# williamyang98/DAB-Radio

Hardware: AMD Instinct MI355X
Metric: dab_mode1_frames_per_sec (higher is better)
Workload: dtype f32

## Files before the change

### dab-radio_amd/csrc/viterbi_lanes.hip

```cpp
#include <hip/hip_runtime.h>
#include <stdint.h>

#include "dabgpu_internal.h"
#include "viterbi_pk16.h"

namespace dabgpu {

__host__ __device__ constexpr int vl_rotl6(int v, int s) { return ((v << s) | (v >> (6 - s))) & 63; }
__host__ __device__ constexpr int vl_idx(int n, int q) { return ((n >> (q + 1)) << q) | (n & ((1 << q) - 1)); }

template <int QN>
__device__ __forceinline__ void vl_gather(const s2 (&D)[32], uint32_t& w0, uint32_t& w1) {
    constexpr int S = (QN + 3) % 6;
    uint32_t G[16];
#pragma unroll
    for (int g = 0; g < 16; g++) {
        const int base = ((g >> 3) << 5) | (g & 7);
        const int r_lo = vl_idx(vl_rotl6(base, S), QN), r_hi = vl_idx(vl_rotl6(base | 16, S), QN);
        G[g] = __builtin_amdgcn_perm(as_u32(D[r_hi]), as_u32(D[r_lo]), 0x0B0A0908u);
    }
    uint32_t a0 = G[0], a1 = G[8];
#pragma unroll
    for (int k = 1; k < 8; k++) {
        a0 = vl_bfi(0x01010101u << k, G[k], a0);
        a1 = vl_bfi(0x01010101u << k, G[8 + k], a1);
    }
    w0 = a0; w1 = a1;
}

template <int Q, int TIE>
__device__ __forceinline__ void vl_step(const s2 (&M)[32], s2 (&N)[32], uint32_t ysym, int k508, uint32_t& w0, uint32_t& w1) {
    s2 C[8], D[32];
    {
        using map = vl_costmap<vl_flip(Q)>;
        constexpr int WF[4] = {map::wF(0, 1, 1, 1), map::wF(1, 1, 1, 1), map::wF(2, 1, 1, 1), map::wF(3, 1, 1, 1)};
        constexpr int WX[4] = {map::wX(0, 1, 1, 1), map::wX(1, 1, 1, 1), map::wX(2, 1, 1, 1), map::wX(3, 1, 1, 1)};
        vl_cost_table<vl_flip(Q), true>(ysym, WF, WX, k508, C);
    }
    if constexpr (Q < 5) {
#pragma unroll
        for (int i = 0; i < 16; i++) {
            const int s = vl_sigma(vl_ins_zero(i, Q));
            const s2 c1 = C[s], c2 = C[7 - s];
            const s2 t1 = addm<TIE>(M[i], c1), t2 = addm<TIE>(M[i + 16], c2);
            const s2 t3 = addm<TIE>(M[i], c2), t4 = addm<TIE>(M[i + 16], c1);
            N[2 * i] = min16(t1, t2);
            N[2 * i + 1] = min16(t3, t4);
            D[2 * i] = TIE ? satsub16(t1, t2) : satsub16(t2, t1);
            D[2 * i + 1] = TIE ? satsub16(t3, t4) : satsub16(t4, t3);
        }
    } else {
#pragma unroll
        for (int b = 0; b < 32; b++) {
            const int s = vl_sigma(b);
            const s2 lower = addm<TIE>(__builtin_shufflevector(M[b], M[b], 0, 0), C[s]);
            const s2 upper = addm<TIE>(__builtin_shufflevector(M[b], M[b], 1, 1), C[7 - s]);
            N[b] = min16(lower, upper);
            D[b] = TIE ? satsub16(lower, upper) : satsub16(upper, lower);
        }
    }
    vl_gather<(Q + 1) % 6>(D, w0, w1);
    if constexpr (TIE != 0) { w0 = ~w0; w1 = ~w1; }
}

__device__ __forceinline__ void vl_renorm(s2 (&N)[32], uint32_t& total) {
    if ((int)N[0].x >= (int)(60455 - 32768)) {
        s2 red[16];
#pragma unroll
        for (int r = 0; r < 16; r++) red[r] = min16(N[r], N[r + 16]);
#pragma unroll
        for (int w = 8; w >= 1; w >>= 1) {
#pragma unroll
            for (int r = 0; r < w; r++) red[r] = min16(red[r], red[r + w]);
        }
        s2 mn = red[0];
        mn = min16(mn, swap16(mn));
        const uint32_t mu = ((uint32_t)(uint16_t)mn.x) ^ 0x8000u;
        const s2 sub = as_s2(mu | (mu << 16));
#pragma unroll
        for (int r = 0; r < 32; r++) N[r] = sub16(N[r], sub);
        total += mu;
    }
}

__device__ __forceinline__ uint2 vl_sched_entry(int t, const uint32_t* seg_pi, const uint32_t* seg_steps, uint32_t in_rows,
                                                const dabgpu_vit_tables* __restrict__ tables) {
    int sstart = 0, in0 = 0, pi = 8, k = 0;
    for (; k < 4; k++) {
        const int len = (int)seg_steps[k];
        if (t < sstart + len) { pi = (int)seg_pi[k]; break; }
        in0 += (len >> 3) * (8 + (int)seg_pi[k]);
        sstart += len;
    }
    const int sis = t - sstart;
    const uint16_t e = tables->pi_tab[pi * 8 + (sis & 7)];
    const uint32_t cnt = e & 0xFFu, kk = (uint32_t)(in0 + (sis >> 3) * (8 + pi)) + (uint32_t)(e >> 8);
    const uint32_t keep = cnt >= 4u ? 0xFFFFFFFFu : ((1u << (8u * cnt)) - 1u);
    uint2 r;
    r.x = min(kk >> 2, in_rows - 2u);
    r.y = ((0x03020100u + (kk & 3u) * 0x01010101u) & keep) | (0x0C0C0C0Cu & ~keep);
    return r;
}

constexpr int VL_OBYTES = 100;

template <int TIE, int VL_WAVES, int OCC = 4>
__global__ __launch_bounds__(64 * VL_WAVES) __attribute__((amdgpu_waves_per_eu(OCC, OCC)))
void vit_lanes_kernel(const dabgpu_vit_group* __restrict__ groups, int n_groups, const dabgpu_cw_desc* __restrict__ descs,
                      const uint32_t* __restrict__ sym, uint32_t* __restrict__ dec, dabgpu_cw_result* __restrict__ results,
                      const dabgpu_vit_tables* __restrict__ tables, const uint2* __restrict__ sched)
{
    __shared__ unsigned char prbs[512];
    __shared__ unsigned short crc_tab[256];
    __shared__ unsigned char obuf[VL_WAVES][64][VL_OBYTES];
    const int lane = threadIdx.x & 63;
    for (int e = threadIdx.x; e < 512; e += 64 * VL_WAVES) prbs[e] = tables->prbs[e];
    for (int e = threadIdx.x; e < 256; e += 64 * VL_WAVES) {
        unsigned v = (unsigned)e << 8;
        for (int qq = 0; qq < 8; qq++) v = (v & 0x8000u) ? (((v << 1) ^ 0x1021u) & 0xFFFFu) : ((v << 1) & 0xFFFFu);
        crc_tab[e] = (unsigned short)v;
    }
    __syncthreads();
    const int wvi = __builtin_amdgcn_readfirstlane((int)(threadIdx.x >> 6));
    const int group = (int)blockIdx.x * VL_WAVES + wvi;
    if (group >= n_groups) return;

    const dabgpu_vit_group Gd = groups[group];
    const int T = (int)Gd.n_steps;
    const bool valid = lane < (int)Gd.count;
    const size_t cw = (size_t)Gd.first + (size_t)Gd.stride * (size_t)(valid ? lane : 0);
    const dabgpu_cw_desc Dd = descs[cw];
    const bool live = valid && Dd.n_steps != 0;

    const uint32_t* grp_sym = sym + Gd.sym_off;
    uint32_t* grp_dec = dec + Gd.dec_off;

    const int q0 = (6 - T % 6) % 6;
    s2 M[32], N[32];
    {
        const uint32_t ss = Dd.start_state & 63u;
        const uint32_t r0 = ((ss >> (q0 + 1)) << q0) | (ss & ((1u << q0) - 1u)), h0 = (ss >> q0) & 1u;
        const uint32_t non = (5080u ^ 0x8000u), st = 0x8000u;
#pragma unroll
        for (int r = 0; r < 32; r++) {
            const uint32_t lo = ((uint32_t)r == r0 && h0 == 0) ? st : non, hi = ((uint32_t)r == r0 && h0 == 1) ? st : non;
            M[r] = as_s2(lo | (hi << 16));
        }
    }
    uint32_t total = 0;
    int k508 = 508;
    asm volatile("" : "+v"(k508));
    const uint2* sch = sched + Gd.sched_off;
    const uint32_t lane4 = 4u * (uint32_t)lane, lane16 = 16u * (uint32_t)lane;
#define VL_PAIR(Q, TT, YA, YB)                                                                        \
    {                                                                                                 \
        uint4 wv;                                                                                     \
        vl_step<Q, TIE>(M, N, YA, k508, wv.x, wv.y);                                                        \
        vl_renorm(N, total);                                                                          \
        vl_step<(Q) + 1, TIE>(N, M, YB, k508, wv.z, wv.w);                                                  \
        vl_renorm(M, total);                                                                          \
        __builtin_nontemporal_store(u4v{wv.x, wv.y, wv.z, wv.w},                                      \
                                    reinterpret_cast<u4v*>(reinterpret_cast<char*>(grp_dec + (size_t)((TT) >> 1) * 256) + lane16)); \
    }
#define VL_ROWS(LO, HI, SEL, TT)                                                                      \
    {                                                                                                 \
        const uint2 e_ = sch[TT];                                                                     \
        const char* rp_ = reinterpret_cast<const char*>(grp_sym + (size_t)e_.x * 64);                 \
        LO = *reinterpret_cast<const uint32_t*>(rp_ + lane4);                                         \
        HI = *reinterpret_cast<const uint32_t*>(rp_ + 256 + lane4);                                   \
        SEL = e_.y;                                                                                   \
    }
    int t = 0;
    if (q0 == 2) {
        uint32_t a0, a1, b0, b1, sa, sb;
        VL_ROWS(a0, a1, sa, t) VL_ROWS(b0, b1, sb, t + 1)
        VL_PAIR(2, t, __builtin_amdgcn_perm(a1, a0, sa), __builtin_amdgcn_perm(b1, b0, sb))
        t += 2;
    }
    if (q0 != 0) {
        uint32_t a0, a1, b0, b1, sa, sb;
        VL_ROWS(a0, a1, sa, t) VL_ROWS(b0, b1, sb, t + 1)
        VL_PAIR(4, t, __builtin_amdgcn_perm(a1, a0, sa), __builtin_amdgcn_perm(b1, b0, sb))
        t += 2;
    }
    uint32_t nlo[6], nhi[6], nsel[6];
#pragma unroll
    for (int q = 0; q < 6; q++) VL_ROWS(nlo[q], nhi[q], nsel[q], t + q)
    for (; t < T; t += 6) {
        uint32_t y[6];
#pragma unroll
        for (int q = 0; q < 6; q++) y[q] = __builtin_amdgcn_perm(nhi[q], nlo[q], nsel[q]);
#pragma unroll
        for (int q = 0; q < 6; q++) VL_ROWS(nlo[q], nhi[q], nsel[q], t + 6 + q)
        VL_PAIR(0, t, y[0], y[1])
        VL_PAIR(2, t + 2, y[2], y[3])
        VL_PAIR(4, t + 4, y[4], y[5])
    }
#undef VL_ROWS
#undef VL_PAIR

    const uint32_t es = Dd.end_state & 63u;
    uint32_t endm = 0;
#pragma unroll
    for (int r = 0; r < 32; r++) endm = ((es >> 1) == (uint32_t)r) ? as_u32(M[r]) : endm;
    endm = (((es & 1u) ? (endm >> 16) : endm) & 0xFFFFu) ^ 0x8000u;

    __builtin_amdgcn_fence(__ATOMIC_RELEASE, "workgroup");
    __builtin_amdgcn_s_waitcnt(0);

    const bool raw = (Dd.flags & DABGPU_CW_RAW) != 0;
    unsigned char* out = reinterpret_cast<unsigned char*>(Dd.d_out);
    const int n_out = (T - 6) >> 3;
    const bool crc_lds = Dd.n_crc_blocks != 0 && n_out <= VL_OBYTES;
    unsigned char* const ob = &obuf[wvi][lane][0];
    uint32_t pos = ((es >> 3) | (es << 3)) & 63u;
    constexpr int CB = 24;
    uint32_t cx[CB], cy[CB];
    for (int th = T - 1; th >= 6; th -= CB) {
#pragma unroll
        for (int v = 0; v < CB / 2; v++) {
            const int pr = (th >> 1) - v;
            const u4v q4 = __builtin_nontemporal_load(reinterpret_cast<const u4v*>(reinterpret_cast<const char*>(grp_dec + (size_t)(pr < 0 ? 0 : pr) * 256) + lane16));
            cx[2 * v] = q4.z; cy[2 * v] = q4.w; cx[2 * v + 1] = q4.x; cy[2 * v + 1] = q4.y;
        }
#pragma unroll
        for (int ub = 0; ub < CB; ub += 8) {
            if (th - ub >= 6) {
                uint32_t acc = 0;
#pragma unroll
                for (int u = ub; u < ub + 8; u++) {
                    const uint32_t word = (pos & 32u) ? cy[u] : cx[u];
                    const uint32_t d = (word >> (pos & 31u)) & 1u;
                    const int b = (3 + u) % 6;
                    pos = (pos & ~(1u << b)) | (d << b);
                    acc |= d << (u - ub);
                }
                const int k = (th - ub - 7 - 6) >> 3;
                const unsigned char pb = raw ? (unsigned char)0 : prbs[k % VL_PRBS];
                if (live) out[k] = (unsigned char)(acc ^ pb);
                if (crc_lds) ob[k] = (unsigned char)(acc ^ pb);
            }
        }
    }

    uint32_t crc_mask = 0;
    if (live && Dd.n_crc_blocks) {
        if (!crc_lds) {
            __builtin_amdgcn_fence(__ATOMIC_RELEASE, "workgroup");
            __builtin_amdgcn_s_waitcnt(0);
        }
        const int blk_bytes = n_out / (int)Dd.n_crc_blocks;
        for (int b = 0; b < (int)Dd.n_crc_blocks && b < 32; b++) {
            unsigned crc = 0xFFFFu, rx;
            if (crc_lds) {
                const unsigned char* fib = ob + b * blk_bytes;
                for (int i = 0; i < blk_bytes - 2; i++) crc = ((crc << 8) ^ crc_tab[((crc >> 8) ^ fib[i]) & 0xFFu]) & 0xFFFFu;
                rx = ((unsigned)fib[blk_bytes - 2] << 8) | fib[blk_bytes - 1];
            } else {
                const unsigned char* fib = out + b * blk_bytes;
                for (int i = 0; i < blk_bytes - 2; i++)
                    crc = ((crc << 8) ^ crc_tab[((crc >> 8) ^ __builtin_nontemporal_load(&fib[i])) & 0xFFu]) & 0xFFFFu;
                rx = ((unsigned)__builtin_nontemporal_load(&fib[blk_bytes - 2]) << 8) | __builtin_nontemporal_load(&fib[blk_bytes - 1]);
            }
            crc ^= 0xFFFFu;
            if (rx == crc) crc_mask |= 1u << b;
        }
    }
    if (valid) {
        dabgpu_cw_result R;
        R.path_error = live ? (uint64_t)total + endm : 0;
        R.crc_ok_mask = crc_mask;
        R.n_out_bytes = live ? (uint32_t)n_out : 0u;
        *reinterpret_cast<dabgpu_cw_result*>(reinterpret_cast<char*>(results + cw) + Gd.res_delta) = R;
    }
}


__device__ __forceinline__ uint32_t vl_clamp4(uint32_t w) {
    const uint32_t t = w ^ 0x80808080u;
    const uint32_t nz = ((t & 0x7F7F7F7Fu) + 0x7F7F7F7Fu) | t;
    return w + ((~nz & 0x80808080u) >> 7);
}

__global__ __launch_bounds__(256)
void vit_prep_kernel(const dabgpu_vit_group* __restrict__ groups, const dabgpu_cw_desc* __restrict__ descs, uint32_t* __restrict__ sym)
{
    __shared__ uint32_t tile[VL_TILE][65];
    const int tid = threadIdx.x, lane = tid & 63, wv = tid >> 6;
    const dabgpu_vit_group Gd = groups[blockIdx.x];
    const int j0 = blockIdx.y * VL_TILE;
    if (j0 >= (int)Gd.in_rows) return;
    const unsigned n_in = dabgpu_vit_in_bytes(Gd.seg_pi, Gd.seg_steps);
    const unsigned i0 = 4u * (unsigned)(j0 + lane);
    for (int c = wv; c < 64; c += 4) {
        uint32_t packed = 0;
        const bool have = c < (int)Gd.count;
        const dabgpu_cw_desc Dd = descs[(size_t)Gd.first + (size_t)Gd.stride * (size_t)(have ? c : 0)];
        uint32_t aoff = 0;
        unsigned ish = 0;
        if (Dd.n_slots != 0) {
            const int age = 15 - (int)(__brev((unsigned)lane & 15u) >> 28);
            int slot = (int)Dd.newest_slot - age;
            if (slot < 0) slot += (int)Dd.n_slots;
            const int fr = slot / (int)Dd.cifs_per_frame, ci = slot - fr * (int)Dd.cifs_per_frame;
            aoff = (uint32_t)fr * Dd.frame_stride + (uint32_t)ci * Dd.cif_stride;
            if (Dd.flags & DABGPU_CW_CLASSED) { aoff += ((unsigned)lane & 15u) * (Dd.cif_stride >> 4); ish = 4; }
        }
        const int8_t* src = reinterpret_cast<const int8_t*>(Dd.d_src);
#pragma unroll
        for (int r = 0; r < 4; r++) {
            const unsigned i = i0 + (unsigned)r;
            const uint32_t off = (uint32_t)__shfl((int)aoff, (int)(i & 15u));
            if (have && Dd.n_steps != 0 && i < n_in) {
                int yv = src[(size_t)off + (i >> ish)];
                yv = max(yv, -127);
                packed |= ((uint32_t)yv & 0xFFu) << (8 * r);
            }
        }
        tile[lane][c] = packed;
    }
    __syncthreads();
    uint32_t* dst = sym + Gd.sym_off;
    for (int s = wv; s < VL_TILE; s += 4) {
        if (j0 + s < (int)Gd.in_rows) dst[(size_t)(j0 + s) * 64 + lane] = tile[s][lane];
    }
}

__global__ __launch_bounds__(256)
void vit_prep_direct_kernel(const dabgpu_vit_group* __restrict__ groups, const dabgpu_cw_desc* __restrict__ descs, uint32_t* __restrict__ sym)
{
    __shared__ uint32_t rows[64][65];
    const int tid = threadIdx.x, lane = tid & 63, wv = tid >> 6;
    const dabgpu_vit_group Gd = groups[blockIdx.x];
    const int j0 = blockIdx.y * VL_TILE;
    if (j0 >= (int)Gd.in_rows) return;
    const int n_in = (int)dabgpu_vit_in_bytes(Gd.seg_pi, Gd.seg_steps);
    typedef const __attribute__((address_space(1))) unsigned char* gptr;
    u4v v[4];
#pragma unroll
    for (int h = 0; h < 4; h++) {
        const int q = tid + 256 * h, c = q >> 4, ch = q & 15;
        v[h] = u4v{0u, 0u, 0u, 0u};
        if (c < (int)Gd.count) {
            const dabgpu_cw_desc* Dd = descs + ((size_t)Gd.first + (size_t)Gd.stride * (size_t)c);
            const int o = 4 * j0 + 16 * ch;
            if (Dd->n_steps != 0 && o < n_in) {
                const gptr p = (gptr)(uintptr_t)Dd->d_src + o;
                if (o + 16 <= n_in) v[h] = *(const __attribute__((address_space(1))) u4v*)p;
                else {
                    const __attribute__((address_space(1))) uint32_t* pw = (const __attribute__((address_space(1))) uint32_t*)p;
                    v[h].x = pw[0];
                    if (o + 8 <= n_in) v[h].y = pw[1];
                    if (o + 12 <= n_in) v[h].z = pw[2];
                }
            }
        }
    }
#pragma unroll
    for (int h = 0; h < 4; h++) {
        const int q = tid + 256 * h, c = q >> 4, ch = q & 15;
        rows[c][4 * ch] = v[h].x; rows[c][4 * ch + 1] = v[h].y; rows[c][4 * ch + 2] = v[h].z; rows[c][4 * ch + 3] = v[h].w;
    }
    __syncthreads();
    uint32_t* dst = sym + Gd.sym_off;
    for (int s = wv; s < VL_TILE; s += 4) {
        if (j0 + s < (int)Gd.in_rows) dst[(size_t)(j0 + s) * 64 + lane] = vl_clamp4(rows[lane][s]);
    }
}

constexpr int VR_ROWS = 19, VR_CHUNKS = 16, VR_PITCH = VR_CHUNKS * 16 + 16;
__global__ __launch_bounds__(256)
void vit_prep_ring4_kernel(const dabgpu_vit_group* __restrict__ groups, const dabgpu_cw_desc* __restrict__ descs, uint32_t* __restrict__ sym)
{
    __shared__ uint32_t tile[VL_TILE][65];
    __shared__ __attribute__((aligned(16))) unsigned char rows[2][VR_ROWS][VR_PITCH];
    const int tid = threadIdx.x, rowi = tid & 63, c = tid >> 6;
    const dabgpu_vit_group Gd = groups[blockIdx.x];
    const int j0 = blockIdx.y * VL_TILE;
    if (j0 >= (int)Gd.in_rows) return;
    const int n_in = (int)dabgpu_vit_in_bytes(Gd.seg_pi, Gd.seg_steps);
    const int i_lo = 4 * j0, i_hi = min(i_lo + 4 * VL_TILE, n_in);
    int lds_off[4];
    bool in[4];
#pragma unroll
    for (int r = 0; r < 4; r++) {
        const unsigned i = (unsigned)(i_lo + 4 * rowi + r);
        const int age = 15 - (int)(__brev(i & 15u) >> 28);
        lds_off[r] = (c - age + 15) * VR_PITCH + (4 * rowi + r);
        in[r] = (int)i < i_hi;
    }
    auto fetch = [&](int k, uint4 (&v)[2]) {
        const bool have = 4 * k < (int)Gd.count;
        const dabgpu_cw_desc Dd = descs[(size_t)Gd.first + (size_t)Gd.stride * (size_t)(have ? 4 * k : 0)];
        const bool on = have && Dd.n_steps != 0;
        const unsigned char* src = reinterpret_cast<const unsigned char*>(Dd.d_src);
#pragma unroll
        for (int h = 0; h < 2; h++) {
            const int q = tid + 256 * h, row = q >> 4, ch = q & 15;
            v[h] = make_uint4(0, 0, 0, 0);
            if (on && row < VR_ROWS && i_lo + 16 * ch < i_hi) {
                int slot = (int)Dd.newest_slot - 15 + row;
                if (slot < 0) slot += (int)Dd.n_slots;
                if (slot >= (int)Dd.n_slots) slot -= (int)Dd.n_slots;
                const size_t off = (size_t)(slot >> 2) * Dd.frame_stride + (size_t)(slot & 3) * Dd.cif_stride + (size_t)(i_lo + 16 * ch);
                v[h] = *reinterpret_cast<const uint4*>(src + off);
            }
        }
    };
    auto stash = [&](int buf, const uint4 (&v)[2]) {
#pragma unroll
        for (int h = 0; h < 2; h++) {
            const int q = tid + 256 * h, row = q >> 4, ch = q & 15;
            if (row < VR_ROWS) *reinterpret_cast<uint4*>(&rows[buf][row][16 * ch]) = v[h];
        }
    };
    uint4 v[4][2];
    fetch(0, v[0]); fetch(1, v[1]); fetch(2, v[2]); fetch(3, v[3]);
    stash(0, v[0]);
    __syncthreads();
#pragma unroll
    for (int k = 0; k < 16; k++) {
        if (k + 4 < 16) fetch(k + 4, v[k & 3]);
        const unsigned char* rb = &rows[k & 1][0][0];
        uint32_t packed = 0;
#pragma unroll
        for (int r = 0; r < 4; r++) {
            if (in[r]) {
                int yv = (int)(signed char)rb[lds_off[r]];
                yv = max(yv, -127);
                packed |= ((uint32_t)yv & 0xFFu) << (8 * r);
            }
        }
        tile[rowi][4 * k + c] = packed;
        if (k + 1 < 16) stash((k + 1) & 1, v[(k + 1) & 3]);
        __syncthreads();
    }
    uint32_t* dst = sym + Gd.sym_off;
    const int lane = tid & 63, wv = tid >> 6;
    for (int s = wv; s < VL_TILE; s += 4) {
        if (j0 + s < (int)Gd.in_rows) dst[(size_t)(j0 + s) * 64 + lane] = tile[s][lane];
    }
}

constexpr int VC_ROWS = 256, VC_ENS = 4;
constexpr int VC_PITCH = 2 * 64 + 16;
constexpr int VC_CIF_PITCH = 16 * VC_PITCH + 16;
constexpr int VC_ENS_PITCH = 4 * VC_CIF_PITCH;
__global__ __launch_bounds__(256)
void vit_prep_ring4c_kernel(const dabgpu_vit_group* __restrict__ groups, const dabgpu_cw_desc* __restrict__ descs, uint32_t* __restrict__ sym,
                            uint32_t groups_per_sub, uint32_t n_lane_sub)
{
    __shared__ __attribute__((aligned(16))) unsigned char ring[VC_ENS * VC_ENS_PITCH];
    const int tid = threadIdx.x;
    unsigned g_idx = blockIdx.x >> 2;
    int qg = (int)(blockIdx.x & 3);
    if (groups_per_sub != 0) {
        const unsigned x = blockIdx.x & 7, j = blockIdx.x >> 3;
        const unsigned li = j % n_lane_sub, u = (j / n_lane_sub) * 8 + x;
        if (u >= 4 * groups_per_sub) return;
        g_idx = li * groups_per_sub + (u >> 2);
        qg = (int)(u & 3);
    }
    const dabgpu_vit_group Gd = groups[g_idx];
    const int n_in = (int)dabgpu_vit_in_bytes(Gd.seg_pi, Gd.seg_steps);
    typedef const __attribute__((address_space(1))) unsigned char* gptr;
    gptr src[VC_ENS];
    unsigned newest[VC_ENS], n_slots = 16, frame_stride = 0, cif_stride = 0;
    bool on[VC_ENS], any = false;
    int phi = 0;
#pragma unroll
    for (int e = 0; e < VC_ENS; e++) {
        const int ens = VC_ENS * qg + e;
        const bool have = 4 * ens < (int)Gd.count;
        const dabgpu_cw_desc Dd = descs[(size_t)Gd.first + (size_t)Gd.stride * (size_t)(have ? 4 * ens : 0)];
        on[e] = have && Dd.n_steps != 0;
        src[e] = (gptr)(uintptr_t)Dd.d_src;
        newest[e] = Dd.newest_slot;
        if (on[e] && !any) {
            any = true; n_slots = Dd.n_slots; frame_stride = Dd.frame_stride; cif_stride = Dd.cif_stride;
            phi = (int)((uintptr_t)Dd.d_src & 63);
        }
    }
    if (!any) return;
    const int piece = tid >> 2, chunk = tid & 3, l_c16 = piece & 15;
    const int l_rel = (piece >> 4) - (15 - (int)(__brev((unsigned)l_c16) >> 28));
    size_t l_off[VC_ENS];
#pragma unroll
    for (int e = 0; e < VC_ENS; e++) {
        int slot = (int)newest[e] + l_rel;
        if (slot < 0) slot += (int)n_slots;
        if (slot >= (int)n_slots) slot -= (int)n_slots;
        l_off[e] = (size_t)(slot >> 2) * frame_stride + (size_t)(slot & 3) * cif_stride + (size_t)l_c16 * (cif_stride >> 4) + (size_t)(16 * chunk) - (size_t)phi;
    }
    unsigned char* const l_lds = ring + (piece >> 4) * VC_CIF_PITCH + l_c16 * VC_PITCH + 16 * chunk;

    const int real_rows = (n_in + 3) >> 2;
    const int n_tiles = (real_rows + VC_ROWS - 1) / VC_ROWS;
    const int last = (((n_in - 1) >> 4) + phi) >> 6;
    auto tile_hi = [&](int st) { return min(st + (phi ? 1 : 0), last); };
    u4v v[VC_ENS];
    auto fetch = [&](int line) {
#pragma unroll
        for (int e = 0; e < VC_ENS; e++) {
            v[e] = u4v{0u, 0u, 0u, 0u};
            if (on[e]) v[e] = *(const __attribute__((address_space(1))) u4v*)(src[e] + (l_off[e] + (size_t)(64 * line)));
        }
    };
    auto stash = [&](int line) {
#pragma unroll
        for (int e = 0; e < VC_ENS; e++) *reinterpret_cast<u4v*>(l_lds + e * VC_ENS_PITCH + (line & 1) * 64) = v[e];
    };
    int loaded = -1;
    bool pend = false;
    const int e = (tid >> 2) & 3, co = tid & 3;
    const uint32_t* const wb = reinterpret_cast<const uint32_t*>(ring) + e * (VC_ENS_PITCH / 4) + co * (VC_CIF_PITCH / 4);
    uint32_t* const obase = sym + Gd.sym_off + 16 * qg + 4 * e + co;
    for (int st = 0; st < n_tiles; st++) {
        if (pend) { stash(loaded); pend = false; }
        while (loaded < tile_hi(st)) { loaded++; fetch(loaded); stash(loaded); }
        __syncthreads();
        if (st + 1 < n_tiles && loaded < tile_hi(st + 1)) { loaded++; fetch(loaded); pend = true; }
#pragma unroll
        for (int it = 0; it < 4; it++) {
            const int m = (tid >> 4) + 16 * it, q = m & 3, cb = m >> 2;
            const int col = (64 * st + 4 * cb + phi) & 127;
            const uint32_t* wp = wb + (4 * q) * (VC_PITCH / 4) + (col >> 2);
            const uint32_t A = wp[0], B = wp[VC_PITCH / 4], C = wp[2 * (VC_PITCH / 4)], D = wp[3 * (VC_PITCH / 4)];
            const uint32_t T0 = __builtin_amdgcn_perm(B, A, 0x05010400u), T1 = __builtin_amdgcn_perm(B, A, 0x07030602u);
            const uint32_t U0 = __builtin_amdgcn_perm(D, C, 0x05010400u), U1 = __builtin_amdgcn_perm(D, C, 0x07030602u);
            const uint32_t O[4] = {__builtin_amdgcn_perm(U0, T0, 0x05040100u), __builtin_amdgcn_perm(U0, T0, 0x07060302u),
                                   __builtin_amdgcn_perm(U1, T1, 0x05040100u), __builtin_amdgcn_perm(U1, T1, 0x07060302u)};
            const int jb = VC_ROWS * st + 16 * cb + q;
#pragma unroll
            for (int mm = 0; mm < 4; mm++) {
                const int j = jb + 4 * mm;
                if (j < real_rows) obase[(size_t)j * 64] = vl_clamp4(O[mm]);
            }
        }
        __syncthreads();
    }
}

__global__ void vit_groups_uniform_kernel(dabgpu_vit_group* groups, size_t n_cw, uint32_t n_steps, uint32_t alloc_steps, uint32_t in_rows,
                                          uint32_t pi0, uint32_t st0, uint32_t pi1, uint32_t st1, uint32_t pi2, uint32_t st2,
                                          uint32_t pi3, uint32_t st3, dabgpu_vit_group_base base)
{
    const size_t g = (size_t)blockIdx.x * blockDim.x + threadIdx.x;
    if (g * 64 >= n_cw) return;
    dabgpu_vit_group G = {};
    G.first = base.first + (uint32_t)(g * 64); G.stride = 1;
    G.count = (uint32_t)((n_cw - g * 64 < 64) ? (n_cw - g * 64) : 64);
    G.n_steps = n_steps; G.alloc_steps = alloc_steps;
    G.seg_pi[0] = pi0; G.seg_steps[0] = st0; G.seg_pi[1] = pi1; G.seg_steps[1] = st1;
    G.seg_pi[2] = pi2; G.seg_steps[2] = st2; G.seg_pi[3] = pi3; G.seg_steps[3] = st3;
    G.in_rows = in_rows;
    G.sched_off = base.sched_off;
    G.sym_off = base.sym_off + g * (size_t)in_rows * 64;
    G.dec_off = base.dec_off + g * (size_t)alloc_steps * 128;
    G.res_delta = base.res_delta;
    groups[g] = G;
}

__global__ void vit_groups_msc_kernel(dabgpu_vit_group* groups, const dabgpu_msc_plan* plans, const uint64_t* lane_subs,
                                      int n_lane_sub, int n_sub, size_t n_ens, uint32_t groups_per_sub, uint32_t sched_stride)
{
    const size_t g = (size_t)blockIdx.x * blockDim.x + threadIdx.x;
    if (g >= (size_t)n_lane_sub * groups_per_sub) return;
    const int li = (int)(g / groups_per_sub);
    const uint32_t gq = (uint32_t)(g - (size_t)li * groups_per_sub);
    const int s = (int)lane_subs[3 * li];
    const dabgpu_msc_plan P = plans[s];
    const size_t n_j = n_ens * 4;
    dabgpu_vit_group G = {};
    G.first = (uint32_t)((size_t)s + (size_t)n_sub * 64 * gq); G.stride = (uint32_t)n_sub;
    G.count = (uint32_t)((n_j - (size_t)gq * 64 < 64) ? (n_j - (size_t)gq * 64) : 64);
    G.n_steps = P.n_steps;
    G.alloc_steps = dabgpu_vit_alloc_steps(P.n_steps);
    for (int k = 0; k < 4; k++) { G.seg_pi[k] = P.seg_pi[k]; G.seg_steps[k] = P.seg_steps[k]; }
    G.in_rows = dabgpu_vit_in_rows(dabgpu_vit_in_bytes(P.seg_pi, P.seg_steps));
    G.sched_off = (uint64_t)li * sched_stride;
    G.sym_off = ((size_t)lane_subs[3 * li + 2] * groups_per_sub + (size_t)gq * G.in_rows) * 64;
    G.dec_off = ((size_t)lane_subs[3 * li + 1] * groups_per_sub + (size_t)gq * G.alloc_steps) * 128;
    groups[g] = G;
}

__global__ void vit_sched_uniform_kernel(uint2* sched, uint32_t sched_stride, uint32_t pi0, uint32_t st0, uint32_t pi1, uint32_t st1,
                                         uint32_t pi2, uint32_t st2, uint32_t pi3, uint32_t st3, const dabgpu_vit_tables* tables)
{
    const uint32_t t = blockIdx.x * blockDim.x + threadIdx.x;
    if (t >= sched_stride) return;
    const uint32_t seg_pi[4] = {pi0, pi1, pi2, pi3}, seg_steps[4] = {st0, st1, st2, st3};
    sched[t] = vl_sched_entry((int)t, seg_pi, seg_steps, dabgpu_vit_in_rows(dabgpu_vit_in_bytes(seg_pi, seg_steps)), tables);
}
__global__ void vit_sched_msc_kernel(uint2* sched, uint32_t sched_stride, const dabgpu_msc_plan* plans, const uint64_t* lane_subs,
                                     const dabgpu_vit_tables* tables)
{
    const uint32_t t = blockIdx.x * blockDim.x + threadIdx.x, li = blockIdx.y;
    if (t >= sched_stride) return;
    const dabgpu_msc_plan P = plans[lane_subs[3 * li]];
    sched[(size_t)li * sched_stride + t] = vl_sched_entry((int)t, P.seg_pi, P.seg_steps, dabgpu_vit_in_rows(dabgpu_vit_in_bytes(P.seg_pi, P.seg_steps)), tables);
}

}

extern "C" hipError_t dabgpu_launch_vit_groups_uniform_at(dabgpu_vit_group* d_groups, size_t n_cw, uint32_t n_steps, const uint32_t* seg_pi,
                                                          const uint32_t* seg_steps, dabgpu_vit_group_base base, hipStream_t stream)
{
    const size_t n_groups = (n_cw + 63) / 64;
    hipLaunchKernelGGL(dabgpu::vit_groups_uniform_kernel, dim3((unsigned)((n_groups + 127) / 128)), dim3(128), 0, stream,
                       d_groups, n_cw, n_steps, dabgpu_vit_alloc_steps(n_steps), dabgpu_vit_in_rows(dabgpu_vit_in_bytes(seg_pi, seg_steps)),
                       seg_pi[0], seg_steps[0], seg_pi[1], seg_steps[1],
                       seg_pi[2], seg_steps[2], seg_pi[3], seg_steps[3], base);
    return hipGetLastError();
}

extern "C" hipError_t dabgpu_launch_vit_groups_uniform(dabgpu_vit_group* d_groups, size_t n_cw, uint32_t n_steps,
                                                       const uint32_t* seg_pi, const uint32_t* seg_steps, hipStream_t stream)
{
    return dabgpu_launch_vit_groups_uniform_at(d_groups, n_cw, n_steps, seg_pi, seg_steps, dabgpu_vit_group_base{0, 0, 0, 0, 0}, stream);
}

extern "C" hipError_t dabgpu_launch_vit_groups_msc(dabgpu_vit_group* d_groups, const dabgpu_msc_plan* d_plans,
                                                   const uint64_t* d_lane_subs, int n_lane_sub, int n_sub, size_t n_ens,
                                                   uint32_t groups_per_sub, uint32_t sched_stride, hipStream_t stream)
{
    const size_t n_groups = (size_t)n_lane_sub * groups_per_sub;
    hipLaunchKernelGGL(dabgpu::vit_groups_msc_kernel, dim3((unsigned)((n_groups + 127) / 128)), dim3(128), 0, stream,
                       d_groups, d_plans, d_lane_subs, n_lane_sub, n_sub, n_ens, groups_per_sub, sched_stride);
    return hipGetLastError();
}

extern "C" hipError_t dabgpu_launch_vit_sched_uniform(uint2* d_sched, uint32_t sched_stride, const uint32_t* seg_pi, const uint32_t* seg_steps,
                                                      const dabgpu_vit_tables* d_tables, hipStream_t stream)
{
    hipLaunchKernelGGL(dabgpu::vit_sched_uniform_kernel, dim3((sched_stride + 255) / 256), dim3(256), 0, stream, d_sched, sched_stride,
                       seg_pi[0], seg_steps[0], seg_pi[1], seg_steps[1], seg_pi[2], seg_steps[2], seg_pi[3], seg_steps[3], d_tables);
    return hipGetLastError();
}

extern "C" hipError_t dabgpu_launch_vit_sched_msc(uint2* d_sched, uint32_t sched_stride, const dabgpu_msc_plan* d_plans,
                                                  const uint64_t* d_lane_subs, int n_lane_sub, const dabgpu_vit_tables* d_tables, hipStream_t stream)
{
    hipLaunchKernelGGL(dabgpu::vit_sched_msc_kernel, dim3((sched_stride + 255) / 256, (unsigned)n_lane_sub), dim3(256), 0, stream, d_sched,
                       sched_stride, d_plans, d_lane_subs, d_tables);
    return hipGetLastError();
}

extern "C" hipError_t dabgpu_launch_vit_prep(int kind, const dabgpu_vit_group* d_groups, size_t n_groups, uint32_t max_in_rows,
                                             const dabgpu_cw_desc* d_descs, uint32_t* d_sym, uint32_t groups_per_sub, hipStream_t stream)
{
    using namespace dabgpu;
    const unsigned tiles = (max_in_rows + VL_TILE - 1) / VL_TILE;
    if (kind == 3)
        hipLaunchKernelGGL(vit_prep_direct_kernel, dim3((unsigned)n_groups, tiles), dim3(256), 0, stream, d_groups, d_descs, d_sym);
    else if (kind == 2)
        if (groups_per_sub != 0 && n_groups % groups_per_sub == 0) {
            const unsigned n_lane_sub = (unsigned)(n_groups / groups_per_sub);
            hipLaunchKernelGGL(vit_prep_ring4c_kernel, dim3(8 * ((4 * groups_per_sub + 7) / 8) * n_lane_sub), dim3(256), 0, stream, d_groups, d_descs,
                               d_sym, groups_per_sub, n_lane_sub);
        } else {
            hipLaunchKernelGGL(vit_prep_ring4c_kernel, dim3((unsigned)(4 * n_groups)), dim3(256), 0, stream, d_groups, d_descs, d_sym, 0u, 1u);
        }
    else if (kind)
        hipLaunchKernelGGL(vit_prep_ring4_kernel, dim3((unsigned)n_groups, tiles), dim3(256), 0, stream, d_groups, d_descs, d_sym);
    else
        hipLaunchKernelGGL(vit_prep_kernel, dim3((unsigned)n_groups, tiles), dim3(256), 0, stream, d_groups, d_descs, d_sym);
    return hipGetLastError();
}

extern "C" hipError_t dabgpu_launch_vit_trellis(const dabgpu_vit_group* d_groups, size_t n_groups, const dabgpu_cw_desc* d_descs, uint32_t* d_sym,
                                                uint32_t* d_dec, dabgpu_cw_result* d_results, int tie_rule, const dabgpu_vit_tables* d_tables,
                                                const uint2* d_sched, int octet, int n_cu, hipStream_t stream)
{
    using namespace dabgpu;
    if (octet) return dabgpu_launch_viterbi_octet(d_groups, n_groups, d_descs, d_sym, d_dec, d_results, tie_rule, d_tables, d_sched, stream);
#define VL_GO(TIE, W) hipLaunchKernelGGL((vit_lanes_kernel<TIE, W>), dim3((unsigned)((n_groups + (W) - 1) / (W))), dim3(64 * (W)), 0, stream, \
                                         d_groups, (int)n_groups, d_descs, d_sym, d_dec, d_results, d_tables, d_sched)
    const bool four = n_groups > (size_t)n_cu && n_groups <= (size_t)4 * n_cu;
    const bool five_per_simd = n_groups > (size_t)16 * n_cu && n_groups <= (size_t)20 * n_cu;
    if (five_per_simd) {
        if (tie_rule) hipLaunchKernelGGL((vit_lanes_kernel<1, 1, 5>), dim3((unsigned)n_groups), dim3(64), 0, stream, d_groups, (int)n_groups, d_descs, d_sym, d_dec, d_results, d_tables, d_sched);
        else hipLaunchKernelGGL((vit_lanes_kernel<0, 1, 5>), dim3((unsigned)n_groups), dim3(64), 0, stream, d_groups, (int)n_groups, d_descs, d_sym, d_dec, d_results, d_tables, d_sched);
    }
    else if (tie_rule) { if (four) VL_GO(1, 4); else VL_GO(1, 1); }
    else { if (four) VL_GO(0, 4); else VL_GO(0, 1); }
#undef VL_GO
    return hipGetLastError();
}
```

### dab-radio_amd/csrc/viterbi_pk16.h

```cpp
#pragma once
#include <hip/hip_runtime.h>
#include <stdint.h>

namespace dabgpu {

typedef short s2 __attribute__((ext_vector_type(2)));
typedef unsigned short us2 __attribute__((ext_vector_type(2)));
typedef unsigned u4v __attribute__((ext_vector_type(4)));

constexpr int VL_TILE = 64;
constexpr int VL_PRBS = 511;

__device__ __forceinline__ uint32_t as_u32(s2 v) { return __builtin_bit_cast(uint32_t, v); }
__device__ __forceinline__ s2 as_s2(uint32_t v) { return __builtin_bit_cast(s2, v); }
__device__ __forceinline__ s2 add16(s2 a, s2 b) { return __builtin_bit_cast(s2, __builtin_bit_cast(us2, a) + __builtin_bit_cast(us2, b)); }
template <int TIE>
__device__ __forceinline__ s2 addm(s2 a, s2 b) {
    if constexpr (TIE != 0) return __builtin_elementwise_add_sat(a, b);
    else return add16(a, b);
}
__device__ __forceinline__ s2 sub16(s2 a, s2 b) { return __builtin_bit_cast(s2, __builtin_bit_cast(us2, a) - __builtin_bit_cast(us2, b)); }
__device__ __forceinline__ s2 min16(s2 a, s2 b) { return __builtin_elementwise_min(a, b); }
__device__ __forceinline__ s2 satsub16(s2 a, s2 b) { return __builtin_elementwise_sub_sat(a, b); }
__device__ __forceinline__ s2 swap16(s2 v) { return __builtin_shufflevector(v, v, 1, 0); }
__device__ __forceinline__ s2 lo_hi(s2 lo_src, s2 hi_src) { return __builtin_shufflevector(lo_src, hi_src, 0, 3); }

__device__ __forceinline__ uint32_t vl_bfi(uint32_t mask, uint32_t a, uint32_t b) {
    uint32_t r;
    asm("v_bfi_b32 %0, %1, %2, %3" : "=v"(r) : "s"(mask), "v"(a), "v"(b));
    return r;
}

__host__ __device__ constexpr int vl_parity(unsigned v) { v ^= v >> 4; v ^= v >> 2; v ^= v >> 1; return (int)(v & 1u); }
__host__ __device__ constexpr int vl_sigma(int b) {
    return vl_parity((2u * (unsigned)b) & 109u) | (vl_parity((2u * (unsigned)b) & 79u) << 1) | (vl_parity((2u * (unsigned)b) & 83u) << 2);
}
__host__ __device__ constexpr int vl_ins_zero(int i, int q) { return ((i >> q) << (q + 1)) | (i & ((1 << q) - 1)); }
__host__ __device__ constexpr int vl_flip(int q) { return q < 5 ? (vl_sigma(0) ^ vl_sigma(1 << q)) : 7; }


template <int FLIP>
struct vl_costmap {
    static_assert(FLIP >= 1 && FLIP <= 7, "pattern difference of the two halves");
    static constexpr int lb = (FLIP & 1) ? 0 : ((FLIP & 2) ? 1 : 2);
    static constexpr int o0 = lb == 0 ? 1 : 0, o1 = lb == 2 ? 1 : 2;
    static constexpr bool f0 = ((FLIP >> o0) & 1) != 0, f1 = ((FLIP >> o1) & 1) != 0;
    static constexpr int nF = 1 << ((f0 ? 1 : 0) + (f1 ? 1 : 0)), nX = 1 << ((f0 ? 0 : 1) + (f1 ? 0 : 1));
    __host__ __device__ static constexpr int idx_of(int s) { const int t = ((s >> lb) & 1) ? s : (s ^ FLIP); return ((t >> o0) & 1) | (((t >> o1) & 1) << 1); }
    __host__ __device__ static constexpr bool swapped(int s) { return ((s >> lb) & 1) == 0; }
    __host__ __device__ static constexpr int fi(int idx) { return f0 ? ((idx & 1) | (f1 ? (idx & 2) : 0)) : (f1 ? ((idx >> 1) & 1) : 0); }
    __host__ __device__ static constexpr int xi(int idx) { return !f0 ? ((idx & 1) | (!f1 ? (idx & 2) : 0)) : (!f1 ? ((idx >> 1) & 1) : 0); }
    __host__ __device__ static constexpr int pack(int wa, int w1, int w2) { return (wa & 0xFF) | ((w1 & 0xFF) << 8) | ((w2 & 0xFF) << 16) | ((wa & 0xFF) << 24); }
    __host__ __device__ static constexpr int wF(int j, int sg0, int sg1, int sg2) {
        int w[3] = {0, 0, 0};
        const int sg[3] = {sg0, sg1, sg2};
        w[lb] = sg[lb];
        int n = 0;
        if (f0) { w[o0] = ((j >> n) & 1) ? sg[o0] : -sg[o0]; n++; }
        if (f1) { w[o1] = ((j >> n) & 1) ? sg[o1] : -sg[o1]; n++; }
        return pack(w[0], w[1], w[2]);
    }
    __host__ __device__ static constexpr int wX(int j, int sg0, int sg1, int sg2) {
        int w[3] = {0, 0, 0};
        const int sg[3] = {sg0, sg1, sg2};
        int n = 0;
        if (!f0) { w[o0] = ((j >> n) & 1) ? -sg[o0] : sg[o0]; n++; }
        if (!f1) { w[o1] = ((j >> n) & 1) ? -sg[o1] : sg[o1]; n++; }
        return pack(w[0], w[1], w[2]);
    }
};

__device__ __forceinline__ s2 vl_cost_reg(int f, int x) {
    uint32_t r;
    const uint32_t signs = 0x0001FFFFu;
    asm("v_pk_mad_i16 %0, %1, %2, %3 op_sel_hi:[0,1,0]" : "=v"(r) : "v"(f), "s"(signs), "v"(x));
    return as_s2(r);
}

template <int NF, int NX, bool WSGPR>
__device__ __forceinline__ void vl_cost_dots(uint32_t y, const int (&WF)[4], const int (&WX)[4], int k508, int (&fv)[4], int (&xv)[4]) {
    static_assert((NF == 1 && NX == 4) || (NF == 2 && NX == 2) || (NF == 4 && NX == 1), "vl_costmap");
    fv[0] = fv[1] = fv[2] = fv[3] = 0; xv[0] = xv[1] = xv[2] = xv[3] = k508;
    if constexpr (NF == 1) {
        if constexpr (WSGPR)
            asm("v_dot4_i32_i8 %0, %5, %6, 0\n\tv_dot4_i32_i8 %1, %5, %7, %11\n\tv_dot4_i32_i8 %2, %5, %8, %11\n\tv_dot4_i32_i8 %3, %5, %9, %11\n\t"
                "v_dot4_i32_i8 %4, %5, %10, %11\n\ts_nop 2"
                : "=&v"(fv[0]), "=&v"(xv[0]), "=&v"(xv[1]), "=&v"(xv[2]), "=&v"(xv[3])
                : "v"(y), "s"(WF[0]), "s"(WX[0]), "s"(WX[1]), "s"(WX[2]), "s"(WX[3]), "v"(k508));
        else
            asm("v_dot4_i32_i8 %0, %5, %6, 0\n\tv_dot4_i32_i8 %1, %5, %7, %11\n\tv_dot4_i32_i8 %2, %5, %8, %11\n\tv_dot4_i32_i8 %3, %5, %9, %11\n\t"
                "v_dot4_i32_i8 %4, %5, %10, %11\n\ts_nop 2"
                : "=&v"(fv[0]), "=&v"(xv[0]), "=&v"(xv[1]), "=&v"(xv[2]), "=&v"(xv[3])
                : "v"(y), "v"(WF[0]), "v"(WX[0]), "v"(WX[1]), "v"(WX[2]), "v"(WX[3]), "v"(k508));
    } else if constexpr (NF == 2) {
        if constexpr (WSGPR)
            asm("v_dot4_i32_i8 %0, %4, %5, 0\n\tv_dot4_i32_i8 %1, %4, %6, 0\n\tv_dot4_i32_i8 %2, %4, %7, %9\n\tv_dot4_i32_i8 %3, %4, %8, %9\n\ts_nop 2"
                : "=&v"(fv[0]), "=&v"(fv[1]), "=&v"(xv[0]), "=&v"(xv[1])
                : "v"(y), "s"(WF[0]), "s"(WF[1]), "s"(WX[0]), "s"(WX[1]), "v"(k508));
        else
            asm("v_dot4_i32_i8 %0, %4, %5, 0\n\tv_dot4_i32_i8 %1, %4, %6, 0\n\tv_dot4_i32_i8 %2, %4, %7, %9\n\tv_dot4_i32_i8 %3, %4, %8, %9\n\ts_nop 2"
                : "=&v"(fv[0]), "=&v"(fv[1]), "=&v"(xv[0]), "=&v"(xv[1])
                : "v"(y), "v"(WF[0]), "v"(WF[1]), "v"(WX[0]), "v"(WX[1]), "v"(k508));
    } else {
        if constexpr (WSGPR)
            asm("v_dot4_i32_i8 %0, %4, %5, 0\n\tv_dot4_i32_i8 %1, %4, %6, 0\n\tv_dot4_i32_i8 %2, %4, %7, 0\n\tv_dot4_i32_i8 %3, %4, %8, 0\n\ts_nop 2"
                : "=&v"(fv[0]), "=&v"(fv[1]), "=&v"(fv[2]), "=&v"(fv[3])
                : "v"(y), "s"(WF[0]), "s"(WF[1]), "s"(WF[2]), "s"(WF[3]));
        else
            asm("v_dot4_i32_i8 %0, %4, %5, 0\n\tv_dot4_i32_i8 %1, %4, %6, 0\n\tv_dot4_i32_i8 %2, %4, %7, 0\n\tv_dot4_i32_i8 %3, %4, %8, 0\n\ts_nop 2"
                : "=&v"(fv[0]), "=&v"(fv[1]), "=&v"(fv[2]), "=&v"(fv[3])
                : "v"(y), "v"(WF[0]), "v"(WF[1]), "v"(WF[2]), "v"(WF[3]));
    }
}

template <int FLIP, bool WSGPR>
__device__ __forceinline__ void vl_cost_table(uint32_t ysym, const int (&WF)[4], const int (&WX)[4], int k508, s2 (&C)[8]) {
    using map = vl_costmap<FLIP>;
    int fv[4], xv[4];
    vl_cost_dots<map::nF, map::nX, WSGPR>(ysym, WF, WX, k508, fv, xv);
    s2 R[4];
#pragma unroll
    for (int i = 0; i < 4; i++) R[i] = vl_cost_reg(fv[map::fi(i)], xv[map::xi(i)]);
#pragma unroll
    for (int s = 0; s < 8; s++) C[s] = map::swapped(s) ? swap16(R[map::idx_of(s)]) : R[map::idx_of(s)];
}

}
```

Before: 2.581 million.

## Split Viterbi decision storage into halves and load only needed half during traceback

Decision words are now stored as two 8-byte halves per lane: the low-32-state words in one 512-byte block and the high-32-state words in another. Traceback no longer loads both halves. It picks the half using the current state's top bit and loads it just in time, every six steps, through a small rolling buffer. This roughly halves traceback read traffic but makes the loads depend on the evolving state, which can expose latency in the serial traceback chain.

```diff
diff --git a/dab-radio_amd/csrc/viterbi_lanes.hip b/dab-radio_amd/csrc/viterbi_lanes.hip
--- a/dab-radio_amd/csrc/viterbi_lanes.hip
+++ b/dab-radio_amd/csrc/viterbi_lanes.hip
@@ -151,7 +151,7 @@
     int k508 = 508;
     asm volatile("" : "+v"(k508));
     const uint2* sch = sched + Gd.sched_off;
-    const uint32_t lane4 = 4u * (uint32_t)lane, lane16 = 16u * (uint32_t)lane;
+    const uint32_t lane4 = 4u * (uint32_t)lane, lane8 = 8u * (uint32_t)lane;
 #define VL_PAIR(Q, TT, YA, YB)                                                                        \
     {                                                                                                 \
         uint4 wv;                                                                                     \
@@ -159,8 +159,9 @@
         vl_renorm(N, total);                                                                          \
         vl_step<(Q) + 1, TIE>(N, M, YB, k508, wv.z, wv.w);                                                  \
         vl_renorm(M, total);                                                                          \
-        __builtin_nontemporal_store(u4v{wv.x, wv.y, wv.z, wv.w},                                      \
-                                    reinterpret_cast<u4v*>(reinterpret_cast<char*>(grp_dec + (size_t)((TT) >> 1) * 256) + lane16)); \
+        char* dp_ = reinterpret_cast<char*>(grp_dec + (size_t)((TT) >> 1) * 256) + lane8;            \
+        __builtin_nontemporal_store(u2v{wv.x, wv.z}, reinterpret_cast<u2v*>(dp_));                    \
+        __builtin_nontemporal_store(u2v{wv.y, wv.w}, reinterpret_cast<u2v*>(dp_ + 512));              \
     }
 #define VL_ROWS(LO, HI, SEL, TT)                                                                      \
     {                                                                                                 \
@@ -215,22 +216,27 @@
     unsigned char* const ob = &obuf[wvi][lane][0];
     uint32_t pos = ((es >> 3) | (es << 3)) & 63u;
     constexpr int CB = 24;
-    uint32_t cx[CB], cy[CB];
+    uint32_t cw_[CB + 3] = {};
+#define VL_DEC(U) (reinterpret_cast<const char*>(grp_dec + (size_t)(((th >> 1) - ((U) >> 1)) < 0 ? 0 : ((th >> 1) - ((U) >> 1))) * 256) + hoff)
+#define VL_LD1(U) cw_[U] = __builtin_nontemporal_load(reinterpret_cast<const uint32_t*>(VL_DEC(U) + (((U) & 1) ? 0 : 4)));
+#define VL_LD2(U) { const u2v q2_ = __builtin_nontemporal_load(reinterpret_cast<const u2v*>(VL_DEC(U))); cw_[U] = q2_.y; cw_[(U) + 1] = q2_.x; }
+    {
+        const int th = T - 1;
+        const uint32_t hoff = lane8 + ((pos & 32u) << 4);
+        VL_LD2(0) VL_LD1(2)
+    }
     for (int th = T - 1; th >= 6; th -= CB) {
-#pragma unroll
-        for (int v = 0; v < CB / 2; v++) {
-            const int pr = (th >> 1) - v;
-            const u4v q4 = __builtin_nontemporal_load(reinterpret_cast<const u4v*>(reinterpret_cast<const char*>(grp_dec + (size_t)(pr < 0 ? 0 : pr) * 256) + lane16));
-            cx[2 * v] = q4.z; cy[2 * v] = q4.w; cx[2 * v + 1] = q4.x; cy[2 * v + 1] = q4.y;
-        }
 #pragma unroll
         for (int ub = 0; ub < CB; ub += 8) {
             if (th - ub >= 6) {
                 uint32_t acc = 0;
 #pragma unroll
                 for (int u = ub; u < ub + 8; u++) {
-                    const uint32_t word = (pos & 32u) ? cy[u] : cx[u];
-                    const uint32_t d = (word >> (pos & 31u)) & 1u;
+                    if (u % 6 == 3) {
+                        const uint32_t hoff = lane8 + ((pos & 32u) << 4);
+                        VL_LD1(u) VL_LD2(u + 1) VL_LD2(u + 3) VL_LD1(u + 5)
+                    }
+                    const uint32_t d = (cw_[u] >> (pos & 31u)) & 1u;
                     const int b = (3 + u) % 6;
                     pos = (pos & ~(1u << b)) | (d << b);
                     acc |= d << (u - ub);
@@ -241,7 +247,11 @@
                 if (crc_lds) ob[k] = (unsigned char)(acc ^ pb);
             }
         }
-    }
+        cw_[0] = cw_[CB]; cw_[1] = cw_[CB + 1]; cw_[2] = cw_[CB + 2];
+    }
+#undef VL_DEC
+#undef VL_LD1
+#undef VL_LD2
 
     uint32_t crc_mask = 0;
     if (live && Dd.n_crc_blocks) {
diff --git a/dab-radio_amd/csrc/viterbi_pk16.h b/dab-radio_amd/csrc/viterbi_pk16.h
--- a/dab-radio_amd/csrc/viterbi_pk16.h
+++ b/dab-radio_amd/csrc/viterbi_pk16.h
@@ -7,6 +7,7 @@
 typedef short s2 __attribute__((ext_vector_type(2)));
 typedef unsigned short us2 __attribute__((ext_vector_type(2)));
 typedef unsigned u4v __attribute__((ext_vector_type(4)));
+typedef unsigned u2v __attribute__((ext_vector_type(2)));
 
 constexpr int VL_TILE = 64;
 constexpr int VL_PRBS = 511;
```

New measurement: 2.574 million. About the same (-0.3%).
